# slp-rl/slamkit

Hardware: NVIDIA H100
Metric: speech-tokens/sec (SLAM seq=1024) (higher is better)
Workload: dtype bf16

## Files before the change

### slamkit_b200/csrc/attention.cu

```cuda
#include "kernels.h"

namespace {

constexpr int HD = 64;

SK_DEVINL uint32_t tile_addr(uint32_t base, int r, int chunk) { return base + r * 128 + ((chunk ^ (r & 7)) << 4); }
SK_DEVINL uint32_t smem_base_1k(const void* p) { return (smem_u32(p) + 1023u) & ~1023u; }

SK_DEVINL void cp_async16(uint32_t saddr, const void* g, bool pred) {
  const int sz = pred ? 16 : 0;
  asm volatile("cp.async.cg.shared.global [%0], [%1], 16, %2;" ::"r"(saddr), "l"(g), "r"(sz) : "memory");
}
SK_DEVINL void cp_async_commit() { asm volatile("cp.async.commit_group;" ::: "memory"); }
template <int N>
SK_DEVINL void cp_async_wait() {
  asm volatile("cp.async.wait_group %0;" ::"n"(N) : "memory");
}

SK_DEVINL void wgmma_m64n64_rs(float (&d)[32], const uint32_t (&a)[4], uint64_t db) {
  asm volatile(
      "{\n\t.reg .pred p;\n\tsetp.eq.u32 p, 1, 1;\n\t"
      "wgmma.mma_async.sync.aligned.m64n64k16.f32.bf16.bf16 {%0,%1,%2,%3,%4,%5,%6,%7,%8,%9,%10,%11,%12,%13,%14,%15,"
      "%16,%17,%18,%19,%20,%21,%22,%23,%24,%25,%26,%27,%28,%29,%30,%31}, {%32,%33,%34,%35}, %36, p, 1, 1, 1;\n\t}\n"
      : "+f"(d[0]), "+f"(d[1]), "+f"(d[2]), "+f"(d[3]), "+f"(d[4]), "+f"(d[5]), "+f"(d[6]), "+f"(d[7]), "+f"(d[8]),
        "+f"(d[9]), "+f"(d[10]), "+f"(d[11]), "+f"(d[12]), "+f"(d[13]), "+f"(d[14]), "+f"(d[15]), "+f"(d[16]),
        "+f"(d[17]), "+f"(d[18]), "+f"(d[19]), "+f"(d[20]), "+f"(d[21]), "+f"(d[22]), "+f"(d[23]), "+f"(d[24]),
        "+f"(d[25]), "+f"(d[26]), "+f"(d[27]), "+f"(d[28]), "+f"(d[29]), "+f"(d[30]), "+f"(d[31])
      : "r"(a[0]), "r"(a[1]), "r"(a[2]), "r"(a[3]), "l"(db));
}

template <int ROWS, int NT>
SK_DEVINL void load_tile(uint32_t sbase, const bf16* g, int ld, int row0, int limit) {
  for (int i = threadIdx.x; i < ROWS * 8; i += NT) {
    const int r = i >> 3, c = i & 7;
    const int gr = row0 + r;
    const bool ok = gr < limit;
    cp_async16(tile_addr(sbase, r, c), g + (size_t)(ok ? gr : 0) * ld + c * 8, ok);
  }
}


SK_DEVINL void wg_a_bT(float (&acc)[8][4], uint32_t sA, uint32_t sB) {
  float(&d)[32] = reinterpret_cast<float(&)[32]>(acc);
  wgmma_fence();
#pragma unroll
  for (int ks = 0; ks < 4; ++ks)
    wgmma_m64n64<0, 0>(d, gmma_desc_sw128(sA + ks * 32, 16, 1024), gmma_desc_sw128(sB + ks * 32, 16, 1024));
  wgmma_commit();
  wgmma_wait<0>();
}

SK_DEVINL void wg_p_b(float (&acc)[8][4], const uint32_t (&p)[4][4], uint32_t sB) {
  float(&d)[32] = reinterpret_cast<float(&)[32]>(acc);
  wgmma_fence();
#pragma unroll
  for (int kk = 0; kk < 4; ++kk) wgmma_m64n64_rs(d, p[kk], gmma_desc_sw128(sB + kk * 2048, 8192, 1024));
  wgmma_commit();
  wgmma_wait<0>();
}

SK_DEVINL void acc_to_a(const float (&s)[8][4], uint32_t (&p)[4][4]) {
#pragma unroll
  for (int kk = 0; kk < 4; ++kk) {
    p[kk][0] = pack_bf16(s[2 * kk][0], s[2 * kk][1]);
    p[kk][1] = pack_bf16(s[2 * kk][2], s[2 * kk][3]);
    p[kk][2] = pack_bf16(s[2 * kk + 1][0], s[2 * kk + 1][1]);
    p[kk][3] = pack_bf16(s[2 * kk + 1][2], s[2 * kk + 1][3]);
  }
}

SK_DEVINL void zero_acc(float (&a)[8][4]) {
#pragma unroll
  for (int i = 0; i < 8; ++i)
#pragma unroll
    for (int j = 0; j < 4; ++j) a[i][j] = 0.f;
}

template <bool CAUSAL>
__global__ void __launch_bounds__(256, 2)
attn_fwd_kernel(const bf16* __restrict__ q, const bf16* __restrict__ k, const bf16* __restrict__ v, bf16* __restrict__ o,
                float* __restrict__ lse, int T, int ld, int ldo, int H, int group, float scale,
                const int* __restrict__ seg_start) {
  extern __shared__ __align__(128) uint8_t smem_attn[];
  const uint32_t sQ = smem_base_1k(smem_attn);
  const uint32_t sK = sQ + 128 * 128;
  const uint32_t sV = sK + 2 * 64 * 128;
  const int b = blockIdx.z, h = blockIdx.y;
  const int qt = gridDim.x - 1 - blockIdx.x;
  const int q0 = qt * 128;
  const int warp = threadIdx.x >> 5, lane = threadIdx.x & 31;
  const bf16* qp = q + (size_t)b * T * ld + h * HD;
  const bf16* kp = k + (size_t)b * T * ld + (h / group) * HD;
  const bf16* vp = v + (size_t)b * T * ld + (h / group) * HD;
  const float sl2 = scale * 1.4426950408889634f;

  int n_kv = (T + 63) / 64;
  if (CAUSAL) {
    const int last = min(T - 1, q0 + 127);
    n_kv = last / 64 + 1;
  }
  load_tile<128, 256>(sQ, qp, ld, q0, T);
  load_tile<64, 256>(sK, kp, ld, 0, T);
  load_tile<64, 256>(sV, vp, ld, 0, T);
  cp_async_commit();

  const uint32_t sQw = sQ + (uint32_t)(warp >> 2) * 8192u;
  float oacc[8][4];
  zero_acc(oacc);
  float m_i[2] = {-INFINITY, -INFINITY}, l_i[2] = {0.f, 0.f};
  const int row_a = q0 + warp * 16 + (lane >> 2);
  int seg_r[2] = {0, 0};
#pragma unroll
  for (int r = 0; r < 2; ++r)
    if (seg_start && row_a + 8 * r < T) seg_r[r] = seg_start[(size_t)b * T + row_a + 8 * r];

  for (int j = 0; j < n_kv; ++j) {
    const int st = j & 1;
    if (j + 1 < n_kv) {
      load_tile<64, 256>(sK + (st ^ 1) * 8192, kp, ld, (j + 1) * 64, T);
      load_tile<64, 256>(sV + (st ^ 1) * 8192, vp, ld, (j + 1) * 64, T);
      cp_async_commit();
      cp_async_wait<1>();
    } else {
      cp_async_wait<0>();
    }
    __syncthreads();

    float s[8][4];
    zero_acc(s);
    wg_a_bT(s, sQw, sK + st * 8192);

    const int k0 = j * 64;
    const bool need_mask = (CAUSAL && (k0 + 63 > q0 + warp * 16)) || (k0 + 64 > T) || seg_start;
    if (need_mask) {
#pragma unroll
      for (int nt = 0; nt < 8; ++nt) {
#pragma unroll
        for (int e = 0; e < 4; ++e) {
          const int key = k0 + nt * 8 + (lane & 3) * 2 + (e & 1);
          const int row = row_a + ((e >> 1) << 3);
          if (key >= T || (CAUSAL && key > row) || key < seg_r[e >> 1]) s[nt][e] = -INFINITY;
        }
      }
    }
    float mx[2] = {m_i[0], m_i[1]};
#pragma unroll
    for (int nt = 0; nt < 8; ++nt) {
      mx[0] = fmaxf(mx[0], fmaxf(s[nt][0], s[nt][1]));
      mx[1] = fmaxf(mx[1], fmaxf(s[nt][2], s[nt][3]));
    }
#pragma unroll
    for (int r = 0; r < 2; ++r) {
      mx[r] = fmaxf(mx[r], __shfl_xor_sync(0xffffffffu, mx[r], 1));
      mx[r] = fmaxf(mx[r], __shfl_xor_sync(0xffffffffu, mx[r], 2));
    }
    float corr[2], rs[2] = {0.f, 0.f};
#pragma unroll
    for (int r = 0; r < 2; ++r) {
      corr[r] = (m_i[r] == -INFINITY) ? 0.f : exp2f((m_i[r] - mx[r]) * sl2);
      m_i[r] = mx[r];
    }
    const float mb0 = (mx[0] == -INFINITY) ? 0.f : mx[0] * sl2;
    const float mb1 = (mx[1] == -INFINITY) ? 0.f : mx[1] * sl2;
#pragma unroll
    for (int nt = 0; nt < 8; ++nt) {
      s[nt][0] = exp2f(s[nt][0] * sl2 - mb0);
      s[nt][1] = exp2f(s[nt][1] * sl2 - mb0);
      s[nt][2] = exp2f(s[nt][2] * sl2 - mb1);
      s[nt][3] = exp2f(s[nt][3] * sl2 - mb1);
      rs[0] += s[nt][0] + s[nt][1];
      rs[1] += s[nt][2] + s[nt][3];
    }
#pragma unroll
    for (int r = 0; r < 2; ++r) l_i[r] = l_i[r] * corr[r] + rs[r];
#pragma unroll
    for (int nt = 0; nt < 8; ++nt) {
      oacc[nt][0] *= corr[0];
      oacc[nt][1] *= corr[0];
      oacc[nt][2] *= corr[1];
      oacc[nt][3] *= corr[1];
    }
    uint32_t pa[4][4];
    acc_to_a(s, pa);
    wg_p_b(oacc, pa, sV + st * 8192);
    __syncthreads();
  }
#pragma unroll
  for (int r = 0; r < 2; ++r) {
    l_i[r] += __shfl_xor_sync(0xffffffffu, l_i[r], 1);
    l_i[r] += __shfl_xor_sync(0xffffffffu, l_i[r], 2);
  }
#pragma unroll
  for (int r = 0; r < 2; ++r) {
    const int row = row_a + 8 * r;
    if (row < T) {
      const float inv = l_i[r] > 0.f ? 1.0f / l_i[r] : 0.f;
      bf16* op = o + ((size_t)b * T + row) * ldo + h * HD;
#pragma unroll
      for (int nt = 0; nt < 8; ++nt) {
        const uint32_t pk = pack_bf16(oacc[nt][2 * r] * inv, oacc[nt][2 * r + 1] * inv);
        *reinterpret_cast<uint32_t*>(op + nt * 8 + (lane & 3) * 2) = pk;
      }
      if (lse && (lane & 3) == 0) lse[((size_t)b * H + h) * T + row] = m_i[r] * scale + logf(l_i[r]);
    }
  }
}

SK_DEVINL void acc_to_a_split(const float (&s)[8][4], uint32_t (&ph)[4][4], uint32_t (&pl)[4][4]) {
#pragma unroll
  for (int kk = 0; kk < 4; ++kk) {
#pragma unroll
    for (int half = 0; half < 2; ++half) {
      const float (&t)[4] = s[2 * kk + half];
      const float h0 = bf16_round(t[0]), h1 = bf16_round(t[1]), h2 = bf16_round(t[2]), h3 = bf16_round(t[3]);
      ph[kk][2 * half] = pack_bf16(h0, h1);
      ph[kk][2 * half + 1] = pack_bf16(h2, h3);
      pl[kk][2 * half] = pack_bf16(t[0] - h0, t[1] - h1);
      pl[kk][2 * half + 1] = pack_bf16(t[2] - h2, t[3] - h3);
    }
  }
}

__global__ void __launch_bounds__(256)
attn_fwd_split_kernel(const bf16* __restrict__ q_hi, const bf16* __restrict__ q_lo, const bf16* __restrict__ k_hi,
                      const bf16* __restrict__ k_lo, const bf16* __restrict__ v_hi, const bf16* __restrict__ v_lo,
                      bf16* __restrict__ o_hi, bf16* __restrict__ o_lo, int T, int ld, int ldo, float scale) {
  extern __shared__ __align__(128) uint8_t smem_attn[];
  const uint32_t sQh = smem_base_1k(smem_attn);
  const uint32_t sQl = sQh + 128 * 128;
  const uint32_t sKV = sQl + 128 * 128;
  const int b = blockIdx.z, h = blockIdx.y;
  const int q0 = blockIdx.x * 128;
  const int warp = threadIdx.x >> 5, lane = threadIdx.x & 31;
  const size_t base = (size_t)b * T * ld + h * HD;
  const float sl2 = scale * 1.4426950408889634f;
  const int n_kv = (T + 63) / 64;

  auto load_kv = [&](int j, int st) {
    const uint32_t sb = sKV + st * 4 * 8192;
    load_tile<64, 256>(sb, k_hi + base, ld, j * 64, T);
    load_tile<64, 256>(sb + 8192, k_lo + base, ld, j * 64, T);
    load_tile<64, 256>(sb + 2 * 8192, v_hi + base, ld, j * 64, T);
    load_tile<64, 256>(sb + 3 * 8192, v_lo + base, ld, j * 64, T);
  };
  load_tile<128, 256>(sQh, q_hi + base, ld, q0, T);
  load_tile<128, 256>(sQl, q_lo + base, ld, q0, T);
  load_kv(0, 0);
  cp_async_commit();

  const uint32_t qh = sQh + (uint32_t)(warp >> 2) * 8192u, ql = sQl + (uint32_t)(warp >> 2) * 8192u;
  float oacc[8][4];
  zero_acc(oacc);
  float m_i[2] = {-INFINITY, -INFINITY}, l_i[2] = {0.f, 0.f};
  const int row_a = q0 + warp * 16 + (lane >> 2);

  for (int j = 0; j < n_kv; ++j) {
    const int st = j & 1;
    if (j + 1 < n_kv) {
      load_kv(j + 1, st ^ 1);
      cp_async_commit();
      cp_async_wait<1>();
    } else {
      cp_async_wait<0>();
    }
    __syncthreads();
    const uint32_t sb = sKV + st * 4 * 8192;
    float s[8][4];
    zero_acc(s);
    wg_a_bT(s, ql, sb);
    wg_a_bT(s, qh, sb + 8192);
    wg_a_bT(s, qh, sb);
    const int k0 = j * 64;
    if (k0 + 64 > T) {
#pragma unroll
      for (int nt = 0; nt < 8; ++nt)
#pragma unroll
        for (int e = 0; e < 4; ++e)
          if (k0 + nt * 8 + (lane & 3) * 2 + (e & 1) >= T) s[nt][e] = -INFINITY;
    }
    float mx[2] = {m_i[0], m_i[1]};
#pragma unroll
    for (int nt = 0; nt < 8; ++nt) {
      mx[0] = fmaxf(mx[0], fmaxf(s[nt][0], s[nt][1]));
      mx[1] = fmaxf(mx[1], fmaxf(s[nt][2], s[nt][3]));
    }
#pragma unroll
    for (int r = 0; r < 2; ++r) {
      mx[r] = fmaxf(mx[r], __shfl_xor_sync(0xffffffffu, mx[r], 1));
      mx[r] = fmaxf(mx[r], __shfl_xor_sync(0xffffffffu, mx[r], 2));
    }
    float corr[2], rs[2] = {0.f, 0.f};
#pragma unroll
    for (int r = 0; r < 2; ++r) {
      corr[r] = (m_i[r] == -INFINITY) ? 0.f : exp2f((m_i[r] - mx[r]) * sl2);
      m_i[r] = mx[r];
    }
    const float mb0 = mx[0] * sl2, mb1 = mx[1] * sl2;
#pragma unroll
    for (int nt = 0; nt < 8; ++nt) {
      s[nt][0] = exp2f(s[nt][0] * sl2 - mb0);
      s[nt][1] = exp2f(s[nt][1] * sl2 - mb0);
      s[nt][2] = exp2f(s[nt][2] * sl2 - mb1);
      s[nt][3] = exp2f(s[nt][3] * sl2 - mb1);
      rs[0] += s[nt][0] + s[nt][1];
      rs[1] += s[nt][2] + s[nt][3];
    }
#pragma unroll
    for (int r = 0; r < 2; ++r) l_i[r] = l_i[r] * corr[r] + rs[r];
#pragma unroll
    for (int nt = 0; nt < 8; ++nt) {
      oacc[nt][0] *= corr[0];
      oacc[nt][1] *= corr[0];
      oacc[nt][2] *= corr[1];
      oacc[nt][3] *= corr[1];
    }
    uint32_t ph[4][4], pl[4][4];
    acc_to_a_split(s, ph, pl);
    wg_p_b(oacc, pl, sb + 2 * 8192);
    wg_p_b(oacc, ph, sb + 3 * 8192);
    wg_p_b(oacc, ph, sb + 2 * 8192);
    __syncthreads();
  }
#pragma unroll
  for (int r = 0; r < 2; ++r) {
    l_i[r] += __shfl_xor_sync(0xffffffffu, l_i[r], 1);
    l_i[r] += __shfl_xor_sync(0xffffffffu, l_i[r], 2);
  }
#pragma unroll
  for (int r = 0; r < 2; ++r) {
    const int row = row_a + 8 * r;
    if (row < T) {
      const float inv = 1.0f / l_i[r];
      const size_t off = ((size_t)b * T + row) * ldo + h * HD;
#pragma unroll
      for (int nt = 0; nt < 8; ++nt) {
        const float v0 = oacc[nt][2 * r] * inv, v1 = oacc[nt][2 * r + 1] * inv;
        const float h0 = bf16_round(v0), h1 = bf16_round(v1);
        *reinterpret_cast<uint32_t*>(o_hi + off + nt * 8 + (lane & 3) * 2) = pack_bf16(h0, h1);
        *reinterpret_cast<uint32_t*>(o_lo + off + nt * 8 + (lane & 3) * 2) = pack_bf16(v0 - h0, v1 - h1);
      }
    }
  }
}

__global__ void attn_delta_kernel(const bf16* __restrict__ o, const bf16* __restrict__ d_o, float* __restrict__ delta,
                                  int B, int T, int H, int ldo) {
  griddep_launch();
  griddep_wait();
  const long total = (long)B * T * H * 8;
  const long i = blockIdx.x * (long)blockDim.x + threadIdx.x;
  const bool ok = i < total;
  float acc = 0.f;
  long rh = 0;
  if (ok) {
    const int part = (int)(i & 7);
    rh = i >> 3;
    const int h = (int)(rh % H);
    const long m = rh / H;
    const uint4 a = ldg128_stream(o + m * ldo + h * HD + part * 8);
    const uint4 g = ldg128_stream(d_o + m * ldo + h * HD + part * 8);
    const uint32_t au[4] = {a.x, a.y, a.z, a.w}, gu[4] = {g.x, g.y, g.z, g.w};
#pragma unroll
    for (int kq = 0; kq < 4; ++kq) {
      const float2 x = unpack_bf16(au[kq]), y = unpack_bf16(gu[kq]);
      acc += x.x * y.x + x.y * y.y;
    }
  }
  acc += __shfl_xor_sync(0xffffffffu, acc, 1);
  acc += __shfl_xor_sync(0xffffffffu, acc, 2);
  acc += __shfl_xor_sync(0xffffffffu, acc, 4);
  if (ok && (i & 7) == 0) {
    const int h = (int)(rh % H);
    const long m = rh / H;
    const long bb = m / T, t = m % T;
    delta[(bb * H + h) * T + t] = acc;
  }
}

template <bool CAUSAL>
__global__ void __launch_bounds__(128, 3)
attn_bwd_dkdv_kernel(const bf16* __restrict__ q, const bf16* __restrict__ k, const bf16* __restrict__ v,
                     const bf16* __restrict__ d_o, const float* __restrict__ lse, const float* __restrict__ delta,
                     bf16* __restrict__ dk, bf16* __restrict__ dv, int T, int ld, int ldo, int ldg, int H, int group,
                     float scale, const int* __restrict__ seg_start) {
  extern __shared__ __align__(128) uint8_t smem_attn[];
  const uint32_t sKV = smem_base_1k(smem_attn);
  const uint32_t sQ = sKV + 2 * 8192;
  const uint32_t sdO = sQ + 2 * 8192;
  float* sStat = reinterpret_cast<float*>(smem_attn + (sKV - smem_u32(smem_attn)) + 6 * 8192);
  int* sSeg = reinterpret_cast<int*>(sStat + 2 * 2 * 64);
  const int b = blockIdx.z, g = blockIdx.y;
  const int kt = blockIdx.x;
  const int k0 = kt * 64;
  const int warp = threadIdx.x >> 5, lane = threadIdx.x & 31;
  const float sl2 = scale * 1.4426950408889634f;
  const bf16* kp = k + (size_t)b * T * ld + g * HD;
  const bf16* vp = v + (size_t)b * T * ld + g * HD;

  load_tile<64, 128>(sKV, kp, ld, k0, T);
  load_tile<64, 128>(sKV + 8192, vp, ld, k0, T);
  cp_async_commit();

  const int n_qt = (T + 63) / 64;
  const int qt_begin = CAUSAL ? kt : 0;
  const int per_head = n_qt - qt_begin;
  const int n_iter = per_head * group;

  auto issue = [&](int it, int st) {
    const int h = g * group + it / per_head;
    const int qt = qt_begin + it % per_head;
    const bf16* qp = q + (size_t)b * T * ld + h * HD;
    const bf16* dop = d_o + (size_t)b * T * ldo + h * HD;
    load_tile<64, 128>(sQ + st * 8192, qp, ld, qt * 64, T);
    load_tile<64, 128>(sdO + st * 8192, dop, ldo, qt * 64, T);
    if (threadIdx.x < 64) {
      const int row = qt * 64 + threadIdx.x;
      const size_t off = ((size_t)b * H + h) * T + (row < T ? row : 0);
      sStat[(st * 2 + 0) * 64 + threadIdx.x] = row < T ? lse[off] : 0.f;
      sStat[(st * 2 + 1) * 64 + threadIdx.x] = row < T ? delta[off] : 0.f;
      sSeg[st * 64 + threadIdx.x] = (seg_start && row < T) ? seg_start[(size_t)b * T + row] : 0;
    }
    cp_async_commit();
  };
  if (n_iter > 0) issue(0, 0);

  float dkacc[8][4], dvacc[8][4];
  zero_acc(dkacc);
  zero_acc(dvacc);
  const int key_a = k0 + warp * 16 + (lane >> 2);

  for (int it = 0; it < n_iter; ++it) {
    const int st = it & 1;
    if (it + 1 < n_iter) {
      issue(it + 1, st ^ 1);
      cp_async_wait<1>();
    } else {
      cp_async_wait<0>();
    }
    __syncthreads();
    const int qt = qt_begin + it % per_head;
    const int q0 = qt * 64;
    const float* s_lse = sStat + (st * 2 + 0) * 64;
    const float* s_del = sStat + (st * 2 + 1) * 64;

    float st_acc[8][4];
    zero_acc(st_acc);
    wg_a_bT(st_acc, sKV, sQ + st * 8192);
    const int* s_seg = sSeg + st * 64;
    const bool need_mask = (CAUSAL && (q0 < k0 + 64)) || (q0 + 64 > T) || (k0 + 64 > T) || seg_start;
#pragma unroll
    for (int nt = 0; nt < 8; ++nt) {
#pragma unroll
      for (int e = 0; e < 4; ++e) {
        const int qi = nt * 8 + (lane & 3) * 2 + (e & 1);
        const int key = key_a + ((e >> 1) << 3);
        float pv = exp2f(st_acc[nt][e] * sl2 - s_lse[qi] * 1.4426950408889634f);
        if (need_mask) {
          const int qrow = q0 + qi;
          if (qrow >= T || key >= T || (CAUSAL && key > qrow) || key < s_seg[qi]) pv = 0.f;
        }
        st_acc[nt][e] = pv;
      }
    }
    uint32_t pa[4][4];
    acc_to_a(st_acc, pa);
    wg_p_b(dvacc, pa, sdO + st * 8192);

    float dp[8][4];
    zero_acc(dp);
    wg_a_bT(dp, sKV + 8192, sdO + st * 8192);
#pragma unroll
    for (int nt = 0; nt < 8; ++nt) {
#pragma unroll
      for (int e = 0; e < 4; ++e) {
        const int qi = nt * 8 + (lane & 3) * 2 + (e & 1);
        dp[nt][e] = st_acc[nt][e] * (dp[nt][e] - s_del[qi]) * scale;
      }
    }
    acc_to_a(dp, pa);
    wg_p_b(dkacc, pa, sQ + st * 8192);
    __syncthreads();
  }
#pragma unroll
  for (int r = 0; r < 2; ++r) {
    const int key = key_a + 8 * r;
    if (key < T) {
      bf16* dkp = dk + ((size_t)b * T + key) * ldg + g * HD;
      bf16* dvp = dv + ((size_t)b * T + key) * ldg + g * HD;
#pragma unroll
      for (int nt = 0; nt < 8; ++nt) {
        *reinterpret_cast<uint32_t*>(dkp + nt * 8 + (lane & 3) * 2) = pack_bf16(dkacc[nt][2 * r], dkacc[nt][2 * r + 1]);
        *reinterpret_cast<uint32_t*>(dvp + nt * 8 + (lane & 3) * 2) = pack_bf16(dvacc[nt][2 * r], dvacc[nt][2 * r + 1]);
      }
    }
  }
}

template <bool CAUSAL>
__global__ void __launch_bounds__(128)
attn_bwd_dq_kernel(const bf16* __restrict__ q, const bf16* __restrict__ k, const bf16* __restrict__ v,
                   const bf16* __restrict__ d_o, const float* __restrict__ lse, const float* __restrict__ delta,
                   bf16* __restrict__ dq, int T, int ld, int ldo, int ldg, int H, int group, float scale,
                   const int* __restrict__ seg_start) {
  extern __shared__ __align__(128) uint8_t smem_attn[];
  const uint32_t sQdO = smem_base_1k(smem_attn);
  const uint32_t sK = sQdO + 2 * 8192;
  const uint32_t sV = sK + 2 * 8192;
  const int b = blockIdx.z, h = blockIdx.y;
  const int qt = gridDim.x - 1 - blockIdx.x;
  const int q0 = qt * 64;
  const int warp = threadIdx.x >> 5, lane = threadIdx.x & 31;
  const float sl2 = scale * 1.4426950408889634f;
  const bf16* qp = q + (size_t)b * T * ld + h * HD;
  const bf16* dop = d_o + (size_t)b * T * ldo + h * HD;
  const bf16* kp = k + (size_t)b * T * ld + (h / group) * HD;
  const bf16* vp = v + (size_t)b * T * ld + (h / group) * HD;

  int n_kv = (T + 63) / 64;
  if (CAUSAL) n_kv = min(T - 1, q0 + 63) / 64 + 1;
  load_tile<64, 128>(sQdO, qp, ld, q0, T);
  load_tile<64, 128>(sQdO + 8192, dop, ldo, q0, T);
  load_tile<64, 128>(sK, kp, ld, 0, T);
  load_tile<64, 128>(sV, vp, ld, 0, T);
  cp_async_commit();

  const int row_a = q0 + warp * 16 + (lane >> 2);
  float lse_r[2], del_r[2];
  int seg_r[2];
#pragma unroll
  for (int r = 0; r < 2; ++r) {
    const int row = row_a + 8 * r;
    const size_t off = ((size_t)b * H + h) * T + (row < T ? row : 0);
    lse_r[r] = row < T ? lse[off] * 1.4426950408889634f : 0.f;
    del_r[r] = row < T ? delta[off] : 0.f;
    seg_r[r] = (seg_start && row < T) ? seg_start[(size_t)b * T + row] : 0;
  }
  float dqacc[8][4];
  zero_acc(dqacc);

  for (int j = 0; j < n_kv; ++j) {
    const int st = j & 1;
    if (j + 1 < n_kv) {
      load_tile<64, 128>(sK + (st ^ 1) * 8192, kp, ld, (j + 1) * 64, T);
      load_tile<64, 128>(sV + (st ^ 1) * 8192, vp, ld, (j + 1) * 64, T);
      cp_async_commit();
      cp_async_wait<1>();
    } else {
      cp_async_wait<0>();
    }
    __syncthreads();
    const int k0 = j * 64;
    float s[8][4];
    zero_acc(s);
    wg_a_bT(s, sQdO, sK + st * 8192);
    const bool need_mask = (CAUSAL && (k0 + 63 > q0 + warp * 16)) || (k0 + 64 > T) || (q0 + 64 > T) || seg_start;
#pragma unroll
    for (int nt = 0; nt < 8; ++nt) {
#pragma unroll
      for (int e = 0; e < 4; ++e) {
        float pv = exp2f(s[nt][e] * sl2 - lse_r[e >> 1]);
        if (need_mask) {
          const int key = k0 + nt * 8 + (lane & 3) * 2 + (e & 1);
          const int row = row_a + ((e >> 1) << 3);
          if (row >= T || key >= T || (CAUSAL && key > row) || key < seg_r[e >> 1]) pv = 0.f;
        }
        s[nt][e] = pv;
      }
    }
    float dp[8][4];
    zero_acc(dp);
    wg_a_bT(dp, sQdO + 8192, sV + st * 8192);
#pragma unroll
    for (int nt = 0; nt < 8; ++nt) {
#pragma unroll
      for (int e = 0; e < 4; ++e) dp[nt][e] = s[nt][e] * (dp[nt][e] - del_r[e >> 1]) * scale;
    }
    uint32_t pa[4][4];
    acc_to_a(dp, pa);
    wg_p_b(dqacc, pa, sK + st * 8192);
    __syncthreads();
  }
#pragma unroll
  for (int r = 0; r < 2; ++r) {
    const int row = row_a + 8 * r;
    if (row < T) {
      bf16* dqp = dq + ((size_t)b * T + row) * ldg + h * HD;
#pragma unroll
      for (int nt = 0; nt < 8; ++nt)
        *reinterpret_cast<uint32_t*>(dqp + nt * 8 + (lane & 3) * 2) = pack_bf16(dqacc[nt][2 * r], dqacc[nt][2 * r + 1]);
    }
  }
}

constexpr int FWD_SMEM = 128 * 128 + 4 * 8192 + 1024;
constexpr int DKDV_SMEM = 6 * 8192 + 2 * 2 * 64 * 4 + 2 * 64 * 4 + 1024;
constexpr int DQ_SMEM = 6 * 8192 + 1024;
constexpr int FWD_SPLIT_SMEM = 2 * 128 * 128 + 8 * 8192 + 1024;

template <typename K>
int set_smem(K kernel, int bytes) {
  SK_CUDA_CHECK(cudaFuncSetAttribute(kernel, cudaFuncAttributeMaxDynamicSharedMemorySize, bytes));
  return 0;
}

}

int sk_attn_fwd_launch(const bf16* q, const bf16* k, const bf16* v, bf16* o, float* lse, int B, int T, int H, int KVH,
                       int ld, int ldo, int causal, float scale, cudaStream_t s, const int* seg_start) {
  SK_REQUIRE(seg_start == nullptr || causal, "attention: document segments need the causal kernel");
  SK_REQUIRE(H % KVH == 0, "attention: H must be a multiple of KVH");
  SK_REQUIRE(ld % 8 == 0 && ldo % 8 == 0, "attention: leading dims must be multiples of 8");
  static bool init = false;
  if (!init) {
    if (set_smem(attn_fwd_kernel<true>, FWD_SMEM)) return -2;
    if (set_smem(attn_fwd_kernel<false>, FWD_SMEM)) return -2;
    init = true;
  }
  dim3 grid((T + 127) / 128, H, B);
  sk_prof_begin(1, s);
  if (causal) attn_fwd_kernel<true><<<grid, 256, FWD_SMEM, s>>>(q, k, v, o, lse, T, ld, ldo, H, H / KVH, scale, seg_start);
  else attn_fwd_kernel<false><<<grid, 256, FWD_SMEM, s>>>(q, k, v, o, lse, T, ld, ldo, H, H / KVH, scale, nullptr);
  sk_prof_end(s);
  SK_LAUNCH_CHECK();
  return 0;
}

int sk_attn_bwd_launch(const bf16* q, const bf16* k, const bf16* v, const bf16* o, const bf16* d_o, const float* lse,
                       float* delta, bf16* dq, bf16* dk, bf16* dv, int B, int T, int H, int KVH, int ld, int ldo,
                       int ldg, int causal, float scale, cudaStream_t s, const int* seg_start) {
  SK_REQUIRE(seg_start == nullptr || causal, "attention: document segments need the causal kernels");
  SK_REQUIRE(H % KVH == 0, "attention: H must be a multiple of KVH");
  static bool init = false;
  if (!init) {
    if (set_smem(attn_bwd_dkdv_kernel<true>, DKDV_SMEM)) return -2;
    if (set_smem(attn_bwd_dkdv_kernel<false>, DKDV_SMEM)) return -2;
    if (set_smem(attn_bwd_dq_kernel<true>, DQ_SMEM)) return -2;
    if (set_smem(attn_bwd_dq_kernel<false>, DQ_SMEM)) return -2;
    init = true;
  }
  const long total = (long)B * T * H * 8;
  sk_prof_begin(1, s);
  SK_CUDA_CHECK(sk_launch_pdl(attn_delta_kernel, dim3((int)((total + 255) / 256)), dim3(256), (size_t)(0), s, o, d_o, delta, B, T, H, ldo));
  SK_LAUNCH_CHECK();
  const int group = H / KVH;
  dim3 g1((T + 63) / 64, KVH, B), g2((T + 63) / 64, H, B);
  if (causal) {
    attn_bwd_dkdv_kernel<true><<<g1, 128, DKDV_SMEM, s>>>(q, k, v, d_o, lse, delta, dk, dv, T, ld, ldo, ldg, H, group, scale,
                                                          seg_start);
    SK_LAUNCH_CHECK();
    attn_bwd_dq_kernel<true><<<g2, 128, DQ_SMEM, s>>>(q, k, v, d_o, lse, delta, dq, T, ld, ldo, ldg, H, group, scale, seg_start);
  } else {
    attn_bwd_dkdv_kernel<false><<<g1, 128, DKDV_SMEM, s>>>(q, k, v, d_o, lse, delta, dk, dv, T, ld, ldo, ldg, H, group, scale,
                                                           nullptr);
    SK_LAUNCH_CHECK();
    attn_bwd_dq_kernel<false><<<g2, 128, DQ_SMEM, s>>>(q, k, v, d_o, lse, delta, dq, T, ld, ldo, ldg, H, group, scale, nullptr);
  }
  sk_prof_end(s);
  SK_LAUNCH_CHECK();
  return 0;
}

int sk_attn_fwd_split_launch(const bf16* q_hi, const bf16* q_lo, const bf16* k_hi, const bf16* k_lo, const bf16* v_hi,
                             const bf16* v_lo, bf16* o_hi, bf16* o_lo, int B, int T, int H, int ld, int ldo, float scale,
                             cudaStream_t s) {
  SK_REQUIRE(ld % 8 == 0 && ldo % 8 == 0, "attention: leading dims must be multiples of 8");
  static bool init = false;
  if (!init) {
    if (set_smem(attn_fwd_split_kernel, FWD_SPLIT_SMEM)) return -2;
    init = true;
  }
  dim3 grid((T + 127) / 128, H, B);
  sk_prof_begin(1, s);
  attn_fwd_split_kernel<<<grid, 256, FWD_SPLIT_SMEM, s>>>(q_hi, q_lo, k_hi, k_lo, v_hi, v_lo, o_hi, o_lo, T, ld, ldo, scale);
  sk_prof_end(s);
  SK_LAUNCH_CHECK();
  return 0;
}

int sk_attn_delta_launch(const bf16* o, const bf16* d_o, float* delta, int B, int T, int H, int ldo, cudaStream_t s) {
  const long total = (long)B * T * H * 8;
  sk_prof_begin(1, s);
  SK_CUDA_CHECK(sk_launch_pdl(attn_delta_kernel, dim3((int)((total + 255) / 256)), dim3(256), (size_t)(0), s, o, d_o, delta, B, T, H, ldo));
  sk_prof_end(s);
  SK_LAUNCH_CHECK();
  return 0;
}

int sk_attn_tc_fwd_launch(const bf16* qkv, bf16* o, float* lse, int B, int T, int H, int KVH, int ld, int ldo, int causal,
                          float scale, cudaStream_t s, const int* seg_start) {
  return sk_attn_fwd_launch(qkv, qkv + H * HD, qkv + (H + KVH) * HD, o, lse, B, T, H, KVH, ld, ldo, causal, scale, s,
                            seg_start);
}

int sk_attn_tc_bwd_launch(const bf16* qkv, const bf16* o, const bf16* d_o, const float* lse, float* delta, float* partial,
                          bf16* dqkv, int B, int T, int H, int KVH, int ld, int ldo, int ldg, int causal, float scale,
                          cudaStream_t s, const int* seg_start, const int* seg_end, const bf16* rope_cos,
                          const bf16* rope_sin, const int* pos_ids, int max_pos) {
  (void)partial;
  SK_REQUIRE((seg_start == nullptr) == (seg_end == nullptr), "attn_tc_bwd: seg_start and seg_end go together");
  SK_REQUIRE((rope_cos == nullptr) == (rope_sin == nullptr) && (rope_cos == nullptr || max_pos > 0), "attn_tc_bwd: rope tables go together");
  int rc = sk_attn_bwd_launch(qkv, qkv + H * HD, qkv + (H + KVH) * HD, o, d_o, lse, delta, dqkv, dqkv + H * HD,
                              dqkv + (H + KVH) * HD, B, T, H, KVH, ld, ldo, ldg, causal, scale, s, seg_start);
  if (rc) return rc;
  if (rope_cos) return sk_rope_launch(dqkv, rope_cos, rope_sin, pos_ids, B * T, T, ldg, H + KVH, HD, 1, max_pos, s);
  return 0;
}

int sk_attn_tc_fwd_split_launch(const bf16* qkv_hi, const bf16* qkv_lo, bf16* o_hi, bf16* o_lo, int B, int T, int H, int ld,
                                int ldo, float scale, cudaStream_t s) {
  return sk_attn_fwd_split_launch(qkv_hi, qkv_lo, qkv_hi + H * HD, qkv_lo + H * HD, qkv_hi + 2 * H * HD, qkv_lo + 2 * H * HD,
                                  o_hi, o_lo, B, T, H, ld, ldo, scale, s);
}
```

### slamkit_b200/csrc/common.cuh

```cuda
#pragma once
#include <cuda_runtime.h>
#include <cuda_bf16.h>
#include <cuda.h>
#include <stdint.h>
#include <stdio.h>

#define SK_DEVINL __device__ __forceinline__

typedef __nv_bfloat16 bf16;
typedef __nv_bfloat162 bf162;

void sk_set_error(const char* fmt, ...);
#define SK_CUDA_CHECK(expr)                                                            \
  do {                                                                                 \
    cudaError_t _e = (expr);                                                           \
    if (_e != cudaSuccess) {                                                           \
      sk_set_error("%s:%d: %s -> %s", __FILE__, __LINE__, #expr, cudaGetErrorString(_e)); \
      return -2;                                                                       \
    }                                                                                  \
  } while (0)
void sk_count_launch();
#define SK_LAUNCH_CHECK()            \
  do {                               \
    sk_count_launch();               \
    SK_CUDA_CHECK(cudaGetLastError()); \
  } while (0)
#define SK_REQUIRE(cond, ...)                  \
  do {                                         \
    if (!(cond)) {                             \
      sk_set_error(__VA_ARGS__);               \
      return -1;                               \
    }                                          \
  } while (0)

int sk_num_sms();

#ifdef __CUDACC__
__device__ __forceinline__ void griddep_wait() { asm volatile("griddepcontrol.wait;" ::: "memory"); }
__device__ __forceinline__ void griddep_launch() { asm volatile("griddepcontrol.launch_dependents;" ::: "memory"); }
#endif
bool sk_pdl_enabled();
template <typename... KArgs, typename... Args>
inline cudaError_t sk_launch_pdl_if(bool pdl, void (*kernel)(KArgs...), dim3 grid, dim3 block, size_t smem, cudaStream_t s,
                                    Args... args) {
  cudaLaunchConfig_t cfg = {};
  cfg.gridDim = grid;
  cfg.blockDim = block;
  cfg.dynamicSmemBytes = smem;
  cfg.stream = s;
  cudaLaunchAttribute attr[1];
  attr[0].id = cudaLaunchAttributeProgrammaticStreamSerialization;
  attr[0].val.programmaticStreamSerializationAllowed = 1;
  cfg.attrs = attr;
  cfg.numAttrs = (pdl && sk_pdl_enabled()) ? 1 : 0;
  return cudaLaunchKernelEx(&cfg, kernel, static_cast<KArgs>(args)...);
}
template <typename... KArgs, typename... Args>
inline cudaError_t sk_launch_pdl(void (*kernel)(KArgs...), dim3 grid, dim3 block, size_t smem, cudaStream_t s, Args... args) {
  return sk_launch_pdl_if(true, kernel, grid, block, smem, s, args...);
}
void sk_prof_begin(int cat, cudaStream_t s);
void sk_prof_end(cudaStream_t s);

SK_DEVINL uint32_t pack_bf16(float lo, float hi) {
  bf162 v = __floats2bfloat162_rn(lo, hi);
  return *reinterpret_cast<uint32_t*>(&v);
}
SK_DEVINL float2 unpack_bf16(uint32_t v) {
  bf162 b = *reinterpret_cast<bf162*>(&v);
  return __bfloat1622float2(b);
}
SK_DEVINL float bf16_round(float x) { return __bfloat162float(__float2bfloat16_rn(x)); }

SK_DEVINL float warp_sum(float v) {
#pragma unroll
  for (int o = 16; o > 0; o >>= 1) v += __shfl_xor_sync(0xffffffffu, v, o);
  return v;
}
SK_DEVINL float warp_max(float v) {
#pragma unroll
  for (int o = 16; o > 0; o >>= 1) v = fmaxf(v, __shfl_xor_sync(0xffffffffu, v, o));
  return v;
}

SK_DEVINL uint4 ldg128(const void* p) { return __ldg(reinterpret_cast<const uint4*>(p)); }
SK_DEVINL uint4 ldg128_stream(const void* p) {
  uint4 r;
  asm volatile("ld.global.nc.L1::no_allocate.v4.u32 {%0,%1,%2,%3}, [%4];"
               : "=r"(r.x), "=r"(r.y), "=r"(r.z), "=r"(r.w)
               : "l"(p));
  return r;
}
SK_DEVINL void stg128(void* p, uint4 v) { *reinterpret_cast<uint4*>(p) = v; }

SK_DEVINL uint32_t smem_u32(const void* p) { return static_cast<uint32_t>(__cvta_generic_to_shared(p)); }

SK_DEVINL uint32_t elect_one() {
  uint32_t pred = 0;
  asm volatile(
      "{\n\t.reg .pred P;\n\t"
      "elect.sync _|P, 0xffffffff;\n\t"
      "selp.u32 %0, 1, 0, P;\n\t}\n"
      : "=r"(pred));
  return pred;
}

SK_DEVINL void mbar_init(uint32_t bar, uint32_t count) {
  asm volatile("mbarrier.init.shared::cta.b64 [%0], %1;" ::"r"(bar), "r"(count) : "memory");
}
SK_DEVINL void fence_mbar_init() { asm volatile("fence.mbarrier_init.release.cluster;" ::: "memory"); }
SK_DEVINL void fence_proxy_async() { asm volatile("fence.proxy.async.shared::cta;" ::: "memory"); }
SK_DEVINL void mbar_arrive(uint32_t bar) {
  asm volatile("mbarrier.arrive.shared::cta.b64 _, [%0];" ::"r"(bar) : "memory");
}
SK_DEVINL void mbar_arrive_expect_tx(uint32_t bar, uint32_t bytes) {
  asm volatile("mbarrier.arrive.expect_tx.shared::cta.b64 _, [%0], %1;" ::"r"(bar), "r"(bytes) : "memory");
}
SK_DEVINL uint32_t mbar_try_wait(uint32_t bar, uint32_t parity) {
  uint32_t ok;
  asm volatile(
      "{\n\t.reg .pred P;\n\t"
      "mbarrier.try_wait.parity.shared::cta.b64 P, [%1], %2;\n\t"
      "selp.u32 %0, 1, 0, P;\n\t}\n"
      : "=r"(ok)
      : "r"(bar), "r"(parity)
      : "memory");
  return ok;
}
SK_DEVINL uint64_t globaltimer_ns() {
  uint64_t t;
  asm volatile("mov.u64 %0, %%globaltimer;" : "=l"(t));
  return t;
}
SK_DEVINL float ex2_approx(float x) {
  float y;
  asm("ex2.approx.ftz.f32 %0, %1;" : "=f"(y) : "f"(x));
  return y;
}

SK_DEVINL float sigmoid_f(float x) {
  float r;
  asm("rcp.approx.ftz.f32 %0, %1;" : "=f"(r) : "f"(1.0f + ex2_approx(x * -1.4426950408889634f)));
  return r;
}
SK_DEVINL float silu_f(float x) { return x * sigmoid_f(x); }

typedef float2 f32x2;
SK_DEVINL f32x2 pk2(float a, float b) { return make_float2(a, b); }
SK_DEVINL void upk2(f32x2 v, float& a, float& b) { a = v.x; b = v.y; }
SK_DEVINL f32x2 dup2(float c) { return make_float2(c, c); }
SK_DEVINL f32x2 fma2(f32x2 a, f32x2 b, f32x2 c) { return make_float2(__fmaf_rn(a.x, b.x, c.x), __fmaf_rn(a.y, b.y, c.y)); }
SK_DEVINL f32x2 mul2(f32x2 a, f32x2 b) { return make_float2(__fmul_rn(a.x, b.x), __fmul_rn(a.y, b.y)); }
SK_DEVINL f32x2 add2(f32x2 a, f32x2 b) { return make_float2(__fadd_rn(a.x, b.x), __fadd_rn(a.y, b.y)); }
SK_DEVINL f32x2 sub2(f32x2 a, f32x2 b) { return make_float2(__fsub_rn(a.x, b.x), __fsub_rn(a.y, b.y)); }
SK_DEVINL void mbar_wait_sleep(uint32_t bar, uint32_t parity) {
  if (mbar_try_wait(bar, parity)) return;
  uint64_t t0 = globaltimer_ns();
  uint32_t spins = 0;
  while (!mbar_try_wait(bar, parity)) {
    __nanosleep(40);
    if ((++spins & 0xfffu) == 0 && globaltimer_ns() - t0 > 4000000000ull) {
      printf("slamkit_b200: mbarrier wait timeout (block %d thread %d bar 0x%x parity %u)\n", blockIdx.x, threadIdx.x, bar,
             parity);
      __trap();
    }
  }
}
SK_DEVINL void mbar_wait(uint32_t bar, uint32_t parity) {
  if (mbar_try_wait(bar, parity)) return;
  uint64_t t0 = globaltimer_ns();
  uint32_t spins = 0;
  while (!mbar_try_wait(bar, parity)) {
    if ((++spins & 0x3fffu) == 0) {
      if (globaltimer_ns() - t0 > 4000000000ull) {
        printf("slamkit_b200: mbarrier wait timeout (block %d thread %d bar 0x%x parity %u)\n", blockIdx.x,
               threadIdx.x, bar, parity);
        __trap();
      }
    }
  }
}

SK_DEVINL void mbar_wait_nocall(uint32_t bar, uint32_t parity) {
  if (mbar_try_wait(bar, parity)) return;
  uint64_t t0 = globaltimer_ns();
  uint32_t spins = 0;
  while (!mbar_try_wait(bar, parity)) {
    if ((++spins & 0x3fffu) == 0 && globaltimer_ns() - t0 > 4000000000ull) __trap();
  }
}

SK_DEVINL void tma_prefetch_desc(const void* tmap) {
  asm volatile("prefetch.tensormap [%0];" ::"l"(tmap) : "memory");
}
SK_DEVINL void tma_load_2d(uint32_t smem_dst, const void* tmap, uint32_t bar, int32_t c0, int32_t c1) {
  asm volatile(
      "cp.async.bulk.tensor.2d.shared::cluster.global.mbarrier::complete_tx::bytes [%0], [%1, {%3, %4}], [%2];"
      ::"r"(smem_dst), "l"(tmap), "r"(bar), "r"(c0), "r"(c1)
      : "memory");
}
SK_DEVINL void tma_load_3d(uint32_t smem_dst, const void* tmap, uint32_t bar, int32_t c0, int32_t c1, int32_t c2) {
  asm volatile(
      "cp.async.bulk.tensor.3d.shared::cluster.global.mbarrier::complete_tx::bytes [%0], [%1, {%3, %4, %5}], [%2];"
      ::"r"(smem_dst), "l"(tmap), "r"(bar), "r"(c0), "r"(c1), "r"(c2)
      : "memory");
}
SK_DEVINL void tma_store_2d(const void* tmap, uint32_t smem_src, int32_t c0, int32_t c1) {
  asm volatile("cp.async.bulk.tensor.2d.global.shared::cta.bulk_group [%0, {%2, %3}], [%1];" ::"l"(tmap),
               "r"(smem_src), "r"(c0), "r"(c1)
               : "memory");
}
SK_DEVINL void tma_store_commit() { asm volatile("cp.async.bulk.commit_group;" ::: "memory"); }
template <int N>
SK_DEVINL void tma_store_wait_read() {
  asm volatile("cp.async.bulk.wait_group.read %0;" ::"n"(N) : "memory");
}
template <int N>
SK_DEVINL void tma_store_wait() {
  asm volatile("cp.async.bulk.wait_group %0;" ::"n"(N) : "memory");
}

SK_DEVINL void wgmma_fence() { asm volatile("wgmma.fence.sync.aligned;" ::: "memory"); }
SK_DEVINL void wgmma_commit() { asm volatile("wgmma.commit_group.sync.aligned;" ::: "memory"); }
template <int N>
SK_DEVINL void wgmma_wait() {
  asm volatile("wgmma.wait_group.sync.aligned %0;" ::"n"(N) : "memory");
}
SK_DEVINL void named_bar_sync(int id, int threads) { asm volatile("bar.sync %0, %1;" ::"r"(id), "r"(threads) : "memory"); }

SK_DEVINL uint64_t gmma_desc_sw128(uint32_t smem_addr, uint32_t lbo_bytes, uint32_t sbo_bytes) {
  uint64_t d = 0;
  d |= (uint64_t)((smem_addr & 0x3ffffu) >> 4);
  d |= (uint64_t)((lbo_bytes >> 4) & 0x3fffu) << 16;
  d |= (uint64_t)((sbo_bytes >> 4) & 0x3fffu) << 32;
  d |= (uint64_t)1 << 62;
  return d;
}
template <int TA, int TB>
SK_DEVINL void wgmma_m64n64(float (&d)[32], uint64_t da, uint64_t db) {
  asm volatile(
      "{\n\t.reg .pred p;\n\tsetp.eq.u32 p, 1, 1;\n\t"
      "wgmma.mma_async.sync.aligned.m64n64k16.f32.bf16.bf16 {%0,%1,%2,%3,%4,%5,%6,%7,%8,%9,%10,%11,%12,%13,%14,%15,%16,%17,%18,%19,%20,%21,%22,%23,%24,%25,%26,%27,%28,%29,%30,%31}, %32, %33, p, 1, 1, %34, %35;\n\t}\n"
      : "+f"(d[0]), "+f"(d[1]), "+f"(d[2]), "+f"(d[3]), "+f"(d[4]), "+f"(d[5]), "+f"(d[6]), "+f"(d[7]), "+f"(d[8]), "+f"(d[9]), "+f"(d[10]), "+f"(d[11]), "+f"(d[12]), "+f"(d[13]), "+f"(d[14]), "+f"(d[15]), "+f"(d[16]), "+f"(d[17]), "+f"(d[18]), "+f"(d[19]), "+f"(d[20]), "+f"(d[21]), "+f"(d[22]), "+f"(d[23]), "+f"(d[24]), "+f"(d[25]), "+f"(d[26]), "+f"(d[27]), "+f"(d[28]), "+f"(d[29]), "+f"(d[30]), "+f"(d[31])
      : "l"(da), "l"(db), "n"(TA), "n"(TB));
}
template <int TA, int TB>
SK_DEVINL void wgmma_m64n128(float (&d)[64], uint64_t da, uint64_t db) {
  asm volatile(
      "{\n\t.reg .pred p;\n\tsetp.eq.u32 p, 1, 1;\n\t"
      "wgmma.mma_async.sync.aligned.m64n128k16.f32.bf16.bf16 {%0,%1,%2,%3,%4,%5,%6,%7,%8,%9,%10,%11,%12,%13,%14,%15,%16,%17,%18,%19,%20,%21,%22,%23,%24,%25,%26,%27,%28,%29,%30,%31,%32,%33,%34,%35,%36,%37,%38,%39,%40,%41,%42,%43,%44,%45,%46,%47,%48,%49,%50,%51,%52,%53,%54,%55,%56,%57,%58,%59,%60,%61,%62,%63}, %64, %65, p, 1, 1, %66, %67;\n\t}\n"
      : "+f"(d[0]), "+f"(d[1]), "+f"(d[2]), "+f"(d[3]), "+f"(d[4]), "+f"(d[5]), "+f"(d[6]), "+f"(d[7]), "+f"(d[8]), "+f"(d[9]), "+f"(d[10]), "+f"(d[11]), "+f"(d[12]), "+f"(d[13]), "+f"(d[14]), "+f"(d[15]), "+f"(d[16]), "+f"(d[17]), "+f"(d[18]), "+f"(d[19]), "+f"(d[20]), "+f"(d[21]), "+f"(d[22]), "+f"(d[23]), "+f"(d[24]), "+f"(d[25]), "+f"(d[26]), "+f"(d[27]), "+f"(d[28]), "+f"(d[29]), "+f"(d[30]), "+f"(d[31]), "+f"(d[32]), "+f"(d[33]), "+f"(d[34]), "+f"(d[35]), "+f"(d[36]), "+f"(d[37]), "+f"(d[38]), "+f"(d[39]), "+f"(d[40]), "+f"(d[41]), "+f"(d[42]), "+f"(d[43]), "+f"(d[44]), "+f"(d[45]), "+f"(d[46]), "+f"(d[47]), "+f"(d[48]), "+f"(d[49]), "+f"(d[50]), "+f"(d[51]), "+f"(d[52]), "+f"(d[53]), "+f"(d[54]), "+f"(d[55]), "+f"(d[56]), "+f"(d[57]), "+f"(d[58]), "+f"(d[59]), "+f"(d[60]), "+f"(d[61]), "+f"(d[62]), "+f"(d[63])
      : "l"(da), "l"(db), "n"(TA), "n"(TB));
}
template <int TA, int TB>
SK_DEVINL void wgmma_m64n256(float (&d)[128], uint64_t da, uint64_t db) {
  asm volatile(
      "{\n\t.reg .pred p;\n\tsetp.eq.u32 p, 1, 1;\n\t"
      "wgmma.mma_async.sync.aligned.m64n256k16.f32.bf16.bf16 {%0,%1,%2,%3,%4,%5,%6,%7,%8,%9,%10,%11,%12,%13,%14,%15,%16,%17,%18,%19,%20,%21,%22,%23,%24,%25,%26,%27,%28,%29,%30,%31,%32,%33,%34,%35,%36,%37,%38,%39,%40,%41,%42,%43,%44,%45,%46,%47,%48,%49,%50,%51,%52,%53,%54,%55,%56,%57,%58,%59,%60,%61,%62,%63,%64,%65,%66,%67,%68,%69,%70,%71,%72,%73,%74,%75,%76,%77,%78,%79,%80,%81,%82,%83,%84,%85,%86,%87,%88,%89,%90,%91,%92,%93,%94,%95,%96,%97,%98,%99,%100,%101,%102,%103,%104,%105,%106,%107,%108,%109,%110,%111,%112,%113,%114,%115,%116,%117,%118,%119,%120,%121,%122,%123,%124,%125,%126,%127}, %128, %129, p, 1, 1, %130, %131;\n\t}\n"
      : "+f"(d[0]), "+f"(d[1]), "+f"(d[2]), "+f"(d[3]), "+f"(d[4]), "+f"(d[5]), "+f"(d[6]), "+f"(d[7]), "+f"(d[8]), "+f"(d[9]), "+f"(d[10]), "+f"(d[11]), "+f"(d[12]), "+f"(d[13]), "+f"(d[14]), "+f"(d[15]), "+f"(d[16]), "+f"(d[17]), "+f"(d[18]), "+f"(d[19]), "+f"(d[20]), "+f"(d[21]), "+f"(d[22]), "+f"(d[23]), "+f"(d[24]), "+f"(d[25]), "+f"(d[26]), "+f"(d[27]), "+f"(d[28]), "+f"(d[29]), "+f"(d[30]), "+f"(d[31]), "+f"(d[32]), "+f"(d[33]), "+f"(d[34]), "+f"(d[35]), "+f"(d[36]), "+f"(d[37]), "+f"(d[38]), "+f"(d[39]), "+f"(d[40]), "+f"(d[41]), "+f"(d[42]), "+f"(d[43]), "+f"(d[44]), "+f"(d[45]), "+f"(d[46]), "+f"(d[47]), "+f"(d[48]), "+f"(d[49]), "+f"(d[50]), "+f"(d[51]), "+f"(d[52]), "+f"(d[53]), "+f"(d[54]), "+f"(d[55]), "+f"(d[56]), "+f"(d[57]), "+f"(d[58]), "+f"(d[59]), "+f"(d[60]), "+f"(d[61]), "+f"(d[62]), "+f"(d[63]), "+f"(d[64]), "+f"(d[65]), "+f"(d[66]), "+f"(d[67]), "+f"(d[68]), "+f"(d[69]), "+f"(d[70]), "+f"(d[71]), "+f"(d[72]), "+f"(d[73]), "+f"(d[74]), "+f"(d[75]), "+f"(d[76]), "+f"(d[77]), "+f"(d[78]), "+f"(d[79]), "+f"(d[80]), "+f"(d[81]), "+f"(d[82]), "+f"(d[83]), "+f"(d[84]), "+f"(d[85]), "+f"(d[86]), "+f"(d[87]), "+f"(d[88]), "+f"(d[89]), "+f"(d[90]), "+f"(d[91]), "+f"(d[92]), "+f"(d[93]), "+f"(d[94]), "+f"(d[95]), "+f"(d[96]), "+f"(d[97]), "+f"(d[98]), "+f"(d[99]), "+f"(d[100]), "+f"(d[101]), "+f"(d[102]), "+f"(d[103]), "+f"(d[104]), "+f"(d[105]), "+f"(d[106]), "+f"(d[107]), "+f"(d[108]), "+f"(d[109]), "+f"(d[110]), "+f"(d[111]), "+f"(d[112]), "+f"(d[113]), "+f"(d[114]), "+f"(d[115]), "+f"(d[116]), "+f"(d[117]), "+f"(d[118]), "+f"(d[119]), "+f"(d[120]), "+f"(d[121]), "+f"(d[122]), "+f"(d[123]), "+f"(d[124]), "+f"(d[125]), "+f"(d[126]), "+f"(d[127])
      : "l"(da), "l"(db), "n"(TA), "n"(TB));
}
template <int N, int TA, int TB>
SK_DEVINL void wgmma_bf16(float (&d)[N / 2], uint64_t da, uint64_t db) {
  if constexpr (N == 256) wgmma_m64n256<TA, TB>(d, da, db);
  else if constexpr (N == 128) wgmma_m64n128<TA, TB>(d, da, db);
  else wgmma_m64n64<TA, TB>(d, da, db);
}
```

Baseline: 119,800.

## Fuse attention backward dK/dV and dQ into one launch and overlap WGMMA groups

Merges the separate dK/dV and dQ backward kernels into a single launch that splits its block index between dK/dV tiles and dQ tiles. This lets the two independent workloads run concurrently and removes one launch boundary. Inside each tile the S and dP wgmma products are now issued as two async groups, so softmax masking on S overlaps the dP matmul. The dV and dK updates are also issued together before a single wait. The dQ tiles now run with the larger dK/dV shared-memory size and the (128,3) launch bound, which may constrain registers or occupancy.

```diff
diff --git a/slamkit_b200/csrc/attention.cu b/slamkit_b200/csrc/attention.cu
--- a/slamkit_b200/csrc/attention.cu
+++ b/slamkit_b200/csrc/attention.cu
@@ -40,23 +40,57 @@
 }
 
 
-SK_DEVINL void wg_a_bT(float (&acc)[8][4], uint32_t sA, uint32_t sB) {
+SK_DEVINL void zero_acc(float (&a)[8][4]) {
+#pragma unroll
+  for (int i = 0; i < 8; ++i)
+#pragma unroll
+    for (int j = 0; j < 4; ++j) a[i][j] = 0.f;
+}
+
+SK_DEVINL void fence_acc(float (&a)[8][4]) {
+#pragma unroll
+  for (int i = 0; i < 8; ++i)
+#pragma unroll
+    for (int j = 0; j < 4; ++j) reg_fence(a[i][j]);
+}
+
+SK_DEVINL void wg_a_bT_issue(float (&acc)[8][4], uint32_t sA, uint32_t sB) {
   float(&d)[32] = reinterpret_cast<float(&)[32]>(acc);
-  wgmma_fence();
 #pragma unroll
   for (int ks = 0; ks < 4; ++ks)
     wgmma_m64n64<0, 0>(d, gmma_desc_sw128(sA + ks * 32, 16, 1024), gmma_desc_sw128(sB + ks * 32, 16, 1024));
+}
+SK_DEVINL void wg_a_bT(float (&acc)[8][4], uint32_t sA, uint32_t sB) {
+  wgmma_fence();
+  wg_a_bT_issue(acc, sA, sB);
   wgmma_commit();
   wgmma_wait<0>();
 }
 
+SK_DEVINL void wg_p_b_issue(float (&acc)[8][4], const uint32_t (&p)[4][4], uint32_t sB) {
+  float(&d)[32] = reinterpret_cast<float(&)[32]>(acc);
+#pragma unroll
+  for (int kk = 0; kk < 4; ++kk) wgmma_m64n64_rs(d, p[kk], gmma_desc_sw128(sB + kk * 2048, 8192, 1024));
+}
 SK_DEVINL void wg_p_b(float (&acc)[8][4], const uint32_t (&p)[4][4], uint32_t sB) {
-  float(&d)[32] = reinterpret_cast<float(&)[32]>(acc);
   wgmma_fence();
-#pragma unroll
-  for (int kk = 0; kk < 4; ++kk) wgmma_m64n64_rs(d, p[kk], gmma_desc_sw128(sB + kk * 2048, 8192, 1024));
+  wg_p_b_issue(acc, p, sB);
   wgmma_commit();
   wgmma_wait<0>();
+}
+
+SK_DEVINL void wg_two_a_bT(float (&a)[8][4], uint32_t sA0, uint32_t sB0, float (&b)[8][4], uint32_t sA1, uint32_t sB1) {
+  zero_acc(a);
+  zero_acc(b);
+  fence_acc(a);
+  fence_acc(b);
+  wgmma_fence();
+  wg_a_bT_issue(a, sA0, sB0);
+  wgmma_commit();
+  wg_a_bT_issue(b, sA1, sB1);
+  wgmma_commit();
+  wgmma_wait<1>();
+  fence_acc(a);
 }
 
 SK_DEVINL void acc_to_a(const float (&s)[8][4], uint32_t (&p)[4][4]) {
@@ -69,12 +103,6 @@
   }
 }
 
-SK_DEVINL void zero_acc(float (&a)[8][4]) {
-#pragma unroll
-  for (int i = 0; i < 8; ++i)
-#pragma unroll
-    for (int j = 0; j < 4; ++j) a[i][j] = 0.f;
-}
 
 template <bool CAUSAL>
 __global__ void __launch_bounds__(256, 2)
@@ -378,19 +406,17 @@
 }
 
 template <bool CAUSAL>
-__global__ void __launch_bounds__(128, 3)
-attn_bwd_dkdv_kernel(const bf16* __restrict__ q, const bf16* __restrict__ k, const bf16* __restrict__ v,
-                     const bf16* __restrict__ d_o, const float* __restrict__ lse, const float* __restrict__ delta,
-                     bf16* __restrict__ dk, bf16* __restrict__ dv, int T, int ld, int ldo, int ldg, int H, int group,
-                     float scale, const int* __restrict__ seg_start) {
+__device__ __forceinline__ void
+attn_bwd_dkdv_tile(const bf16* __restrict__ q, const bf16* __restrict__ k, const bf16* __restrict__ v,
+                   const bf16* __restrict__ d_o, const float* __restrict__ lse, const float* __restrict__ delta,
+                   bf16* __restrict__ dk, bf16* __restrict__ dv, int T, int ld, int ldo, int ldg, int H, int group,
+                   float scale, const int* __restrict__ seg_start, int kt, int g, int b) {
   extern __shared__ __align__(128) uint8_t smem_attn[];
   const uint32_t sKV = smem_base_1k(smem_attn);
   const uint32_t sQ = sKV + 2 * 8192;
   const uint32_t sdO = sQ + 2 * 8192;
   float* sStat = reinterpret_cast<float*>(smem_attn + (sKV - smem_u32(smem_attn)) + 6 * 8192);
   int* sSeg = reinterpret_cast<int*>(sStat + 2 * 2 * 64);
-  const int b = blockIdx.z, g = blockIdx.y;
-  const int kt = blockIdx.x;
   const int k0 = kt * 64;
   const int warp = threadIdx.x >> 5, lane = threadIdx.x & 31;
   const float sl2 = scale * 1.4426950408889634f;
@@ -443,9 +469,8 @@
     const float* s_lse = sStat + (st * 2 + 0) * 64;
     const float* s_del = sStat + (st * 2 + 1) * 64;
 
-    float st_acc[8][4];
-    zero_acc(st_acc);
-    wg_a_bT(st_acc, sKV, sQ + st * 8192);
+    float st_acc[8][4], dp[8][4];
+    wg_two_a_bT(st_acc, sKV, sQ + st * 8192, dp, sKV + 8192, sdO + st * 8192);
     const int* s_seg = sSeg + st * 64;
     const bool need_mask = (CAUSAL && (q0 < k0 + 64)) || (q0 + 64 > T) || (k0 + 64 > T) || seg_start;
 #pragma unroll
@@ -462,13 +487,8 @@
         st_acc[nt][e] = pv;
       }
     }
-    uint32_t pa[4][4];
-    acc_to_a(st_acc, pa);
-    wg_p_b(dvacc, pa, sdO + st * 8192);
-
-    float dp[8][4];
-    zero_acc(dp);
-    wg_a_bT(dp, sKV + 8192, sdO + st * 8192);
+    wgmma_wait<0>();
+    fence_acc(dp);
 #pragma unroll
     for (int nt = 0; nt < 8; ++nt) {
 #pragma unroll
@@ -477,8 +497,16 @@
         dp[nt][e] = st_acc[nt][e] * (dp[nt][e] - s_del[qi]) * scale;
       }
     }
-    acc_to_a(dp, pa);
-    wg_p_b(dkacc, pa, sQ + st * 8192);
+    uint32_t pa[4][4], dsa[4][4];
+    acc_to_a(st_acc, pa);
+    acc_to_a(dp, dsa);
+    wgmma_fence();
+    wg_p_b_issue(dvacc, pa, sdO + st * 8192);
+    wg_p_b_issue(dkacc, dsa, sQ + st * 8192);
+    wgmma_commit();
+    wgmma_wait<0>();
+    fence_acc(dvacc);
+    fence_acc(dkacc);
     __syncthreads();
   }
 #pragma unroll
@@ -497,17 +525,15 @@
 }
 
 template <bool CAUSAL>
-__global__ void __launch_bounds__(128)
-attn_bwd_dq_kernel(const bf16* __restrict__ q, const bf16* __restrict__ k, const bf16* __restrict__ v,
+__device__ __forceinline__ void
+attn_bwd_dq_tile(const bf16* __restrict__ q, const bf16* __restrict__ k, const bf16* __restrict__ v,
                    const bf16* __restrict__ d_o, const float* __restrict__ lse, const float* __restrict__ delta,
                    bf16* __restrict__ dq, int T, int ld, int ldo, int ldg, int H, int group, float scale,
-                   const int* __restrict__ seg_start) {
+                   const int* __restrict__ seg_start, int qt, int h, int b) {
   extern __shared__ __align__(128) uint8_t smem_attn[];
   const uint32_t sQdO = smem_base_1k(smem_attn);
   const uint32_t sK = sQdO + 2 * 8192;
   const uint32_t sV = sK + 2 * 8192;
-  const int b = blockIdx.z, h = blockIdx.y;
-  const int qt = gridDim.x - 1 - blockIdx.x;
   const int q0 = qt * 64;
   const int warp = threadIdx.x >> 5, lane = threadIdx.x & 31;
   const float sl2 = scale * 1.4426950408889634f;
@@ -550,9 +576,8 @@
     }
     __syncthreads();
     const int k0 = j * 64;
-    float s[8][4];
-    zero_acc(s);
-    wg_a_bT(s, sQdO, sK + st * 8192);
+    float s[8][4], dp[8][4];
+    wg_two_a_bT(s, sQdO, sK + st * 8192, dp, sQdO + 8192, sV + st * 8192);
     const bool need_mask = (CAUSAL && (k0 + 63 > q0 + warp * 16)) || (k0 + 64 > T) || (q0 + 64 > T) || seg_start;
 #pragma unroll
     for (int nt = 0; nt < 8; ++nt) {
@@ -567,9 +592,8 @@
         s[nt][e] = pv;
       }
     }
-    float dp[8][4];
-    zero_acc(dp);
-    wg_a_bT(dp, sQdO + 8192, sV + st * 8192);
+    wgmma_wait<0>();
+    fence_acc(dp);
 #pragma unroll
     for (int nt = 0; nt < 8; ++nt) {
 #pragma unroll
@@ -592,9 +616,32 @@
   }
 }
 
+template <bool CAUSAL>
+__global__ void __launch_bounds__(128, 3)
+attn_bwd_kernel(const bf16* __restrict__ q, const bf16* __restrict__ k, const bf16* __restrict__ v,
+                const bf16* __restrict__ d_o, const float* __restrict__ lse, const float* __restrict__ delta,
+                bf16* __restrict__ dq, bf16* __restrict__ dk, bf16* __restrict__ dv, int B, int T, int ld, int ldo, int ldg,
+                int H, int group, float scale, const int* __restrict__ seg_start) {
+  const int n_t = (T + 63) / 64, KVH = H / group;
+  const int n_dkdv = n_t * KVH * B;
+  int i = blockIdx.x;
+  if (i < n_dkdv) {
+    const int kt = i / (KVH * B);
+    i -= kt * KVH * B;
+    attn_bwd_dkdv_tile<CAUSAL>(q, k, v, d_o, lse, delta, dk, dv, T, ld, ldo, ldg, H, group, scale, seg_start, kt, i % KVH,
+                               i / KVH);
+  } else {
+    i -= n_dkdv;
+    const int qt = n_t - 1 - i / (H * B);
+    i %= H * B;
+    attn_bwd_dq_tile<CAUSAL>(q, k, v, d_o, lse, delta, dq, T, ld, ldo, ldg, H, group, scale, seg_start, qt, i % H, i / H);
+  }
+}
+
 constexpr int FWD_SMEM = 128 * 128 + 4 * 8192 + 1024;
 constexpr int DKDV_SMEM = 6 * 8192 + 2 * 2 * 64 * 4 + 2 * 64 * 4 + 1024;
 constexpr int DQ_SMEM = 6 * 8192 + 1024;
+static_assert(DQ_SMEM <= DKDV_SMEM, "the fused backward launch sizes its shared memory for the dK/dV CTAs");
 constexpr int FWD_SPLIT_SMEM = 2 * 128 * 128 + 8 * 8192 + 1024;
 
 template <typename K>
@@ -632,10 +679,8 @@
   SK_REQUIRE(H % KVH == 0, "attention: H must be a multiple of KVH");
   static bool init = false;
   if (!init) {
-    if (set_smem(attn_bwd_dkdv_kernel<true>, DKDV_SMEM)) return -2;
-    if (set_smem(attn_bwd_dkdv_kernel<false>, DKDV_SMEM)) return -2;
-    if (set_smem(attn_bwd_dq_kernel<true>, DQ_SMEM)) return -2;
-    if (set_smem(attn_bwd_dq_kernel<false>, DQ_SMEM)) return -2;
+    if (set_smem(attn_bwd_kernel<true>, DKDV_SMEM)) return -2;
+    if (set_smem(attn_bwd_kernel<false>, DKDV_SMEM)) return -2;
     init = true;
   }
   const long total = (long)B * T * H * 8;
@@ -643,18 +688,14 @@
   SK_CUDA_CHECK(sk_launch_pdl(attn_delta_kernel, dim3((int)((total + 255) / 256)), dim3(256), (size_t)(0), s, o, d_o, delta, B, T, H, ldo));
   SK_LAUNCH_CHECK();
   const int group = H / KVH;
-  dim3 g1((T + 63) / 64, KVH, B), g2((T + 63) / 64, H, B);
-  if (causal) {
-    attn_bwd_dkdv_kernel<true><<<g1, 128, DKDV_SMEM, s>>>(q, k, v, d_o, lse, delta, dk, dv, T, ld, ldo, ldg, H, group, scale,
-                                                          seg_start);
-    SK_LAUNCH_CHECK();
-    attn_bwd_dq_kernel<true><<<g2, 128, DQ_SMEM, s>>>(q, k, v, d_o, lse, delta, dq, T, ld, ldo, ldg, H, group, scale, seg_start);
-  } else {
-    attn_bwd_dkdv_kernel<false><<<g1, 128, DKDV_SMEM, s>>>(q, k, v, d_o, lse, delta, dk, dv, T, ld, ldo, ldg, H, group, scale,
-                                                           nullptr);
-    SK_LAUNCH_CHECK();
-    attn_bwd_dq_kernel<false><<<g2, 128, DQ_SMEM, s>>>(q, k, v, d_o, lse, delta, dq, T, ld, ldo, ldg, H, group, scale, nullptr);
-  }
+  const long n_blocks = (long)((T + 63) / 64) * (KVH + H) * B;
+  SK_REQUIRE(n_blocks <= 0x7fffffff, "attention: too many tiles for one launch");
+  if (causal)
+    attn_bwd_kernel<true><<<(unsigned)n_blocks, 128, DKDV_SMEM, s>>>(q, k, v, d_o, lse, delta, dq, dk, dv, B, T, ld, ldo, ldg,
+                                                                     H, group, scale, seg_start);
+  else
+    attn_bwd_kernel<false><<<(unsigned)n_blocks, 128, DKDV_SMEM, s>>>(q, k, v, d_o, lse, delta, dq, dk, dv, B, T, ld, ldo,
+                                                                      ldg, H, group, scale, nullptr);
   sk_prof_end(s);
   SK_LAUNCH_CHECK();
   return 0;
diff --git a/slamkit_b200/csrc/common.cuh b/slamkit_b200/csrc/common.cuh
--- a/slamkit_b200/csrc/common.cuh
+++ b/slamkit_b200/csrc/common.cuh
@@ -227,6 +227,8 @@
   asm volatile("wgmma.wait_group.sync.aligned %0;" ::"n"(N) : "memory");
 }
 SK_DEVINL void named_bar_sync(int id, int threads) { asm volatile("bar.sync %0, %1;" ::"r"(id), "r"(threads) : "memory"); }
+SK_DEVINL void reg_fence(float& x) { asm volatile("" : "+f"(x)::"memory"); }
+
 
 SK_DEVINL uint64_t gmma_desc_sw128(uint32_t smem_addr, uint32_t lbo_bytes, uint32_t sbo_bytes) {
   uint64_t d = 0;
```

New measurement: 123,100 (median of 6 runs). +2.8%, better.
